# LukasHaas/PIGEON

Hardware: AMD Instinct MI355X
Metric: images/sec end-to-end (ViT+head+refine), 4x336x336 (higher is better)
Workload: dtype f16

## Files before the change

### include/pigeon_hip.h

```cpp
#ifndef PIGEON_HIP_H
#define PIGEON_HIP_H

#include <stddef.h>
#include <stdint.h>

#ifdef __cplusplus
extern "C" {
#endif

#define PG_OK            0
#define PG_EINVAL       -1
#define PG_ENOMEM       -2
#define PG_EHIP         -3
#define PG_ESTATE       -4

#define PG_DTYPE_F32     0
#define PG_DTYPE_BF16    1
#define PG_DTYPE_F16     2
#define PG_DTYPE_F64     3

#define PG_ABI_VERSION   7

const char* pg_last_error(void);
int pg_abi_version(void);
// ... 82 lines not shown
int pg_refine_forward(const pg_bank* bank, const float* q, int B, int P, const double* init_llh,
                      const int64_t* cand, const float* cand_prob, int k, int topk,
                      float temperature, double max_refine_km, float* scratch,
                      float* out_llh, int64_t* out_cell, int32_t* out_choice, void* stream);

int pg_refine_forward_ex(const pg_bank* bank, const float* q, int B, int P, const double* init_llh,
                         const int64_t* cand, const float* cand_prob, int k, int topk, int n_eval,
                         float temperature, double max_refine_km, float* scratch12,
                         float* out_llh, int64_t* out_cell, int32_t* out_choice, int32_t* out_refined, void* stream);

int pg_refine_certainty(const pg_bank* bank, const float* q, int B, int P, const int64_t* cand, const float* cand_prob, int k,
                        int topk, int n_eval, const float* scratch12, const float* W, int C, const float* beta,
                        const float* wstats, float temperature, const int32_t* refined, const int32_t* choice,
                        float* tol, int32_t* code, void* stream);

int pg_requeue_append(const float* head_tol, const float* refine_tol, const int32_t* refine_code, int B, float thr, int force_all,
                      int64_t dst_base, int64_t flushed, int64_t cap, int64_t* counters, int64_t* slot_dst, int32_t* row_slot,
                      uint8_t* certain, int32_t* cause, void* stream);
int pg_rows_to_slots(const void* src, int64_t row_bytes, const int32_t* row_slot, int B, void* dst, void* stream);
int pg_requeue_take(const int64_t* slot_dst, int64_t cap, int64_t head, int n_valid, int n_pad, int64_t* dst_out, void* stream);
int pg_scatter_rows(const void* src, int64_t row_bytes, const int64_t* dst_row, int n, void* dst, int64_t dst_rows,
                    int64_t remap_wb, int64_t remap_b, int64_t remap_off, void* stream);
int pg_head_wstats(const float* W, int C, const float* beta, float* out2, void* stream);

int pg_embedding_debias(float* emb, int64_t n, int dim, const float* bias, void* stream);

typedef struct pg_prep pg_prep;
int pg_prep_create(pg_prep** out, int device, int in_h, int in_w);
int pg_prep_destroy(pg_prep* h);
int pg_prep_geometry(const pg_prep* h, int32_t* out6);
int pg_prep_workspace_bytes(const pg_prep* h, int n_images, size_t* bytes);
int pg_prep_forward(pg_prep* h, const void* images_u8, int n_images, void* out, int out_dtype, void* workspace,
                    size_t workspace_bytes, void* stream);

#define PG_PREP_ITEM_BYTES 80
#define PG_PREP_RAGGED_MAX_IMAGES 65535
typedef struct pg_prep_item {
    uint64_t src_off;
    int32_t in_h, in_w;
    int32_t new_h, new_w, top, left;
    int32_t ksize_h, ksize_v;
    int32_t row0, nrows;
    int32_t tmp_row;
    uint32_t bounds_h_off, kk_h_off, bounds_v_off, kk_v_off;
    int32_t reserved[3];
} pg_prep_item;
// ... 65 lines not shown
```

### pigeon_amd/_lib.py

```python
from __future__ import annotations

import ctypes as C
import os

_HERE = os.path.dirname(os.path.abspath(__file__))
LIB_PATH = os.environ.get("PIGEON_HIP_LIB") or os.path.join(_HERE, "libpigeon_hip.so")

PG_DTYPE_F32, PG_DTYPE_BF16, PG_DTYPE_F16, PG_DTYPE_F64 = 0, 1, 2, 3
EPI_QKV, EPI_GELU, EPI_RESID, EPI_PATCH, EPI_F32, EPI_RESID_STAT, EPI_QKV_LN, EPI_GELU_LN, EPI_GELU_X3 = 0, 1, 2, 3, 4, 5, 6, 7, 8
PROF_CLASSES = ["gemm_qkv", "gemm_out", "gemm_fc1", "gemm_fc2", "gemm_patch", "attention", "layernorm",
                "im2col", "token_mean"]


class PigeonHipError(RuntimeError):
    pass


class VitCfg(C.Structure):
    _fields_ = [("layers", C.c_int32), ("image_size", C.c_int32), ("patch", C.c_int32), ("hidden", C.c_int32),
                ("heads", C.c_int32), ("mlp", C.c_int32), ("ln_eps", C.c_float), ("max_chunk", C.c_int32),
                ("mma_dtype", C.c_int32), ("precise", C.c_int32)]


class Bank(C.Structure):
    _fields_ = [("proto_emb", C.c_void_p), ("cell_off", C.c_void_p), ("proto_lnglat", C.c_void_p),
                ("proto_count", C.c_void_p), ("member_off", C.c_void_p), ("member_idx", C.c_void_p),
                ("train_emb", C.c_void_p), ("train_lnglat", C.c_void_p),
                ("num_cells", C.c_int64), ("num_protos", C.c_int64), ("num_train", C.c_int64)]


class PrepItem(C.Structure):
    _fields_ = [("src_off", C.c_uint64), ("in_h", C.c_int32), ("in_w", C.c_int32), ("new_h", C.c_int32), ("new_w", C.c_int32),
                ("top", C.c_int32), ("left", C.c_int32), ("ksize_h", C.c_int32), ("ksize_v", C.c_int32), ("row0", C.c_int32),
                ("nrows", C.c_int32), ("tmp_row", C.c_int32), ("bounds_h_off", C.c_uint32), ("kk_h_off", C.c_uint32),
                ("bounds_v_off", C.c_uint32), ("kk_v_off", C.c_uint32), ("reserved", C.c_int32 * 3)]


PREP_ITEM_BYTES = 80
assert C.sizeof(PrepItem) == PREP_ITEM_BYTES


_P, _I, _I64, _F, _D, _SZ = C.c_void_p, C.c_int, C.c_int64, C.c_float, C.c_double, C.c_size_t
SIGNATURES = {
    "pg_last_error": (C.c_char_p, []),
    "pg_abi_version": (_I, []),
    "pg_device_count": (_I, []),
    "pg_vit_create": (_I, [C.POINTER(_P), _I, C.POINTER(VitCfg)]),
    "pg_vit_load_weight": (_I, [_P, C.c_char_p, _P, _I, C.POINTER(_I64), _I]),
    "pg_vit_finalize": (_I, [_P]),
    "pg_vit_workspace_bytes": (_I, [_P, _I, C.POINTER(_SZ)]),
    "pg_vit_forward": (_I, [_P, _P, _I, _I, _P, _P, _SZ, _P]),
    "pg_vit_forward_hidden": (_I, [_P, _P, _I, _I, _P, _P, _P, _SZ, _P]),
    "pg_vit_precise_workspace_bytes": (_I, [_P, _I, C.POINTER(_SZ)]),
    "pg_vit_forward_precise": (_I, [_P, _P, _I, _I, _P, _P, _P, _SZ, _P]),
    "pg_vit_graph": (_I, [_P, _I, C.POINTER(_I64), C.POINTER(_I64)]),
    "pg_vit_destroy": (_I, [_P]),
    "pg_vit_mma_dtype": (_I, [_P]),
    "pg_fingerprint": (_I, [_P, _SZ, C.c_uint64, C.POINTER(C.c_uint64), _P]),
    "pg_vit_fingerprint": (_I, [_P, C.POINTER(C.c_uint64)]),
    "pg_vit_profile_enable": (_I, [_P, _I]),
    "pg_vit_profile_read": (_I, [_P, C.POINTER(_I64), C.POINTER(_D)]),
    "pg_vit_profile_reset": (_I, [_P]),
# ... 25 lines not shown
    "pg_prep_ragged_create": (_I, [C.POINTER(_P), _I]),
    "pg_prep_ragged_destroy": (_I, [_P]),
    "pg_prep_ragged_forward": (_I, [_P, _P, _SZ, C.POINTER(PrepItem), _I, _P, _I, _P, _SZ, _P]),
    "pg_proto_build": (_I, [_P, _I, _I64, _P, _P, _I64, _P, _P]),
    "pg_haversine_matrix": (_I, [_P, _I, _P, _I, _I, _P, _P]),
    "pg_haversine_pairs": (_I, [_P, _P, _I, _I64, _P, _P]),
    "pg_smooth_labels": (_I, [_P, _I, _I, _D, _P, _P]),
    "pg_haversine_blocks": (_I, [_P, _P, _P, _I, _D, _P, _P]),
    "pg_optics_graph": (_I, [_P, _P, _P, _I, _I, _P, _P, _P, _P, _P]),
    "pg_optics_plan": (_I, [_I64, _I, C.POINTER(C.c_int32)]),
    "pg_tune_optics_lds_points": (_I, [_I]),
    "pg_head_forward": (_I, [_P, _I, _I, _P, _P, _P, _I, _I, _P, _P, _P, _P, _P, _P]),
    "pg_head_margin": (_I, [_P, _I, _I, _P, _I, _P, _P, _P, _P, _P]),
    "pg_head_certainty": (_I, [_P, _I, _I, _P, _I, _P, _P, _I, _P, _P, _P, _P, _P, _P, _P]),
    "pg_aux_heads_forward": (_I, [_P, _I, _I, _P, _P, _I, _I, _I, _P, _P, _P, _P, _P, _P, _P]),
    "pg_refine_forward": (_I, [C.POINTER(Bank), _P, _I, _I, _P, _P, _P, _I, _I, _F, _D, _P, _P, _P, _P, _P]),
    "pg_refine_forward_ex": (_I, [C.POINTER(Bank), _P, _I, _I, _P, _P, _P, _I, _I, _I, _F, _D, _P, _P, _P, _P, _P, _P]),
    "pg_refine_certainty": (_I, [C.POINTER(Bank), _P, _I, _I, _P, _P, _I, _I, _I, _P, _P, _I, _P, _P, _F, _P, _P, _P, _P, _P]),
    "pg_requeue_append": (_I, [_P, _P, _P, _I, _F, _I, _I64, _I64, _I64, _P, _P, _P, _P, _P, _P]),
    "pg_rows_to_slots": (_I, [_P, _I64, _P, _I, _P, _P]),
    "pg_requeue_take": (_I, [_P, _I64, _I64, _I, _I, _P, _P]),
    "pg_scatter_rows": (_I, [_P, _I64, _P, _I, _P, _I64, _I64, _I64, _I64, _P]),
    "pg_head_wstats": (_I, [_P, _I, _P, _P, _P]),
    "pg_embedding_debias": (_I, [_P, _I64, _I, _P, _P]),
    "pg_op_gemm16": (_I, [_I, _P, _I64, _P, _P, _P, _I64, _I, _I, _I, _I, _F, _I, _P, _I, _P]),
    "pg_op_gemm16_ld": (_I, [_I, _P, _I64, _P, _I64, _P, _P, _I64, _I, _I, _I, _I, _F, _I, _P, _I, _P]),
    "pg_op_rowstat_cast": (_I, [_P, _P, _I, _P, _I64, _F, _P]),
    "pg_op_gemm16_resid_stat": (_I, [_I, _P, _I64, _P, _I64, _P, _P, _I64, _P, _I64, _P, _I, _I, _I, _I, _P]),
    "pg_op_rowstat_finalize": (_I, [_P, _I, _P, _I64, _F, _P]),
    "pg_op_gemm16_ln": (_I, [_I, _P, _I64, _P, _I64, _P, _P, _P, _P, _I64, _I, _I, _I, _I, _F, _I, _I, _P]),
    "pg_op_layernorm": (_I, [_P, _P, _P, _P, _I, _I64, _F, _P]),
    "pg_op_attention": (_I, [_I, _P, _P, _I, _P]),
    "pg_op_im2col": (_I, [_P, _I, _P, _I, _I, _P]),
    "pg_op_token_mean": (_I, [_P, _P, _I, _P]),
    "pg_op_cast_f32": (_I, [_P, _P, _I, _I64, _P]),
    "pg_op_gemm16_parts": (_I, [_I, _P, _I64, _P, _I64, _P, _P, _I, _I, _I, _I, _P]),
    "pg_op_x3_split": (_I, [_P, _P, _I64, _I, _I, _P]),
    "pg_op_x3_layernorm": (_I, [_P, _P, _P, _P, _I64, _F, _P]),
    "pg_op_attention_f32": (_I, [_P, _P, _I, _P]),
    "pg_op_attention_x3": (_I, [_P, _P, _I, _P]),
    "pg_op_x3_im2col": (_I, [_P, _I, _P, _I, _P]),
    "pg_op_sum_parts": (_I, [_P, _I, _I64, _P, _I64, _I, _P]),
    "pg_op_preln": (_I, [_P, _P, _P, _P, _P, _I64, _F, _P, _I, _P, _P]),
    "pg_vit_precise_plan": (_I, [_I, C.POINTER(C.c_int32)]),
}

# ... 35 lines not shown
```

### pigeon_amd/csrc/head.hip

```cpp
#include "common.h"
#include "pigeon_internal.h"
#include "certainty_common.h"
#include <cfloat>

#define HT 64
#define HK 32

__global__ __launch_bounds__(256) void head_logits_kernel(const float* __restrict__ emb, int B, int P,
                                                          const float* __restrict__ W, const float* __restrict__ bias,
                                                          int C, float* __restrict__ logits) {
    __shared__ float As[HK][HT + 1];
    __shared__ float Ws[HK][HT + 1];
    const int tid = threadIdx.x;
    const int c0 = blockIdx.x * HT, b0 = blockIdx.y * HT;
    const int tx = tid & 15, ty = tid >> 4;
    float acc[4][4];
#pragma unroll
    for (int i = 0; i < 4; ++i)
#pragma unroll
        for (int j = 0; j < 4; ++j) acc[i][j] = 0.f;
    const float invP = 1.0f / (float)P;
    for (int k0 = 0; k0 < VIT_HIDDEN; k0 += HK) {
#pragma unroll
        for (int i = 0; i < 8; ++i) {
            const int idx = tid + i * 256;
            const int r = idx >> 5, k = idx & 31;
            float a = 0.f;
            if (b0 + r < B) {
                const float* e = emb + ((int64_t)(b0 + r) * P) * VIT_HIDDEN + k0 + k;
                for (int p = 0; p < P; ++p) a += e[(int64_t)p * VIT_HIDDEN];
                a *= invP;
            }
            As[k][r] = a;
            Ws[k][r] = (c0 + r < C) ? W[(int64_t)(c0 + r) * VIT_HIDDEN + k0 + k] : 0.f;
        }
        __syncthreads();
#pragma unroll
        for (int k = 0; k < HK; ++k) {
            float a[4], w[4];
#pragma unroll
            for (int i = 0; i < 4; ++i) a[i] = As[k][ty * 4 + i];
#pragma unroll
            for (int j = 0; j < 4; ++j) w[j] = Ws[k][tx * 4 + j];
#pragma unroll
            for (int i = 0; i < 4; ++i)
#pragma unroll
                for (int j = 0; j < 4; ++j) acc[i][j] = fmaf(a[i], w[j], acc[i][j]);
        }
        __syncthreads();
    }
#pragma unroll
    for (int i = 0; i < 4; ++i) {
        const int b = b0 + ty * 4 + i;
        if (b >= B) continue;
#pragma unroll
        for (int j = 0; j < 4; ++j) {
            const int c = c0 + tx * 4 + j;
            if (c < C) logits[(int64_t)b * C + c] = acc[i][j] + bias[c];
        }
    }
}

struct ValIdx { float v; int i; };
__device__ __forceinline__ ValIdx block_argbest(ValIdx x, ValIdx* red ) {
#pragma unroll
    for (int o = 32; o >= 1; o >>= 1) {
        const float ov = __shfl_xor(x.v, o, 64);
        const int oi = __shfl_xor(x.i, o, 64);
        if (better(ov, oi, x.v, x.i)) { x.v = ov; x.i = oi; }
    }
    const int wave = threadIdx.x >> 6;
    __syncthreads();
    if ((threadIdx.x & 63) == 0) red[wave] = x;
    __syncthreads();
    ValIdx r = red[0];
#pragma unroll
    for (int w = 1; w < 4; ++w) if (better(red[w].v, red[w].i, r.v, r.i)) r = red[w];
    return r;
}

template <bool GLOBAL>
// ... 35 lines not shown
            topk_val[(int64_t)b * k + r] = best.v;
            topk_idx[(int64_t)b * k + r] = best.i;
            if (r == 0) {
                argmax_out[b] = best.i;
                pred_llh[2 * b] = centroids[2 * (int64_t)best.i];
                pred_llh[2 * b + 1] = centroids[2 * (int64_t)best.i + 1];
            }
            probs[best.i] = -2.f;
        }
        if (GLOBAL) __threadfence_block();
        __syncthreads();
    }
}

extern "C" int pg_head_forward(const float* emb, int B, int P, const float* W, const float* bias,
                               const double* centroids, int C, int k, float* logits, float* topk_val,
                               int64_t* topk_idx, int64_t* argmax, double* pred_llh, void* stream) {
    hipStream_t s = (hipStream_t)stream;
    if (B < 0) { pg_set_error("head: B = %d", B); return PG_EINVAL; }
    if (B == 0) return PG_OK;
    if (!emb || !W || !bias || !centroids || !logits || !topk_val || !topk_idx || !argmax || !pred_llh) {
        pg_set_error("head: null pointer argument"); return PG_EINVAL;
    }
    if (P < 1 || C < 1 || k < 1 || k > C) { pg_set_error("head: bad P=%d C=%d k=%d", P, C, k); return PG_EINVAL; }
    const size_t lds = (size_t)C * sizeof(float);
    const bool big = lds > 150 * 1024;
    dim3 g1((C + HT - 1) / HT, (B + HT - 1) / HT);
    hipLaunchKernelGGL(head_logits_kernel, g1, dim3(256), 0, s, emb, B, P, W, bias, C, logits);
    int rc = pg_check_launch("head_logits");
    if (rc) return rc;
    if (big) {
        float* scratch = nullptr;
        PG_HIP(hipMallocAsync((void**)&scratch, (size_t)B * C * sizeof(float), s));
        hipLaunchKernelGGL(head_row_kernel<true>, dim3(B), dim3(256), 0, s, logits, C, k, centroids, topk_val, topk_idx, argmax, pred_llh, scratch);
        rc = pg_check_launch("head_row (large C)");
        (void)hipFreeAsync(scratch, s);
        return rc;
    }
    static size_t attr_lds = 0;
    if (lds > attr_lds) {
        PG_HIP(hipFuncSetAttribute((const void*)head_row_kernel<false>, hipFuncAttributeMaxDynamicSharedMemorySize, (int)lds));
        attr_lds = lds;
    }
    hipLaunchKernelGGL(head_row_kernel<false>, dim3(B), dim3(256), lds, s, logits, C, k, centroids, topk_val, topk_idx, argmax, pred_llh,
                       (float*)nullptr);
    return pg_check_launch("head_row");
}

__global__ __launch_bounds__(256) void head_margin_kernel(const float* __restrict__ logits, int C, const float* __restrict__ emb, int P,
                                                          const float* __restrict__ W, float* __restrict__ margin,
                                                          float* __restrict__ sens, int64_t* __restrict__ top2) {
// ... 56 lines not shown
```

### pigeon_amd/csrc/requeue.hip

```cpp
#include "common.h"
#include "pigeon_internal.h"

namespace {

__global__ void __launch_bounds__(256)
requeue_append_kernel(const float* __restrict__ head_tol, const float* __restrict__ refine_tol, const int32_t* __restrict__ refine_code,
                      int B, float thr, int force_all, int64_t dst_base, int64_t flushed, int64_t cap,
                      int64_t* __restrict__ counters, int64_t* __restrict__ slot_dst, int32_t* __restrict__ row_slot,
                      uint8_t* __restrict__ certain, int32_t* __restrict__ cause) {
    __shared__ int wave_cnt[4];
    __shared__ int64_t s_app, s_drop;
    const int tid = threadIdx.x, lane = tid & 63, wv = tid >> 6;
    if (tid == 0) { s_app = counters ? counters[0] : 0; s_drop = counters ? counters[1] : 0; }
    __syncthreads();
    for (int base = 0; base < B; base += 256) {
        const int r = base + tid;
        bool flag = false;
        int why = 0;
        if (r < B) {
            const bool h_unc = force_all || !(head_tol[r] > thr);
            const bool r_unc = refine_tol ? !(refine_tol[r] > thr) : false;
            flag = h_unc || r_unc;
            why = h_unc ? 1 : (r_unc ? (refine_code ? refine_code[r] : 2) : 0);
            if (r_unc && !h_unc && why == 0) why = 2;
// ... 74 lines not shown
head_wstats_kernel(const float* __restrict__ W, int C, const float* __restrict__ beta, unsigned int* __restrict__ out) {
    const int lane = threadIdx.x & 63;
    const int c = blockIdx.x * 4 + (threadIdx.x >> 6);
    if (c >= C) return;
    const float* row = W + (int64_t)c * 1024;
    float n2 = 0.f, wb = 0.f;
#pragma unroll
    for (int i = 0; i < 4; ++i) {
        const f32x4 v = *(const f32x4*)(row + i * 256 + lane * 4);
        n2 = fmaf(v[0], v[0], fmaf(v[1], v[1], fmaf(v[2], v[2], fmaf(v[3], v[3], n2))));
        if (beta) {
            const f32x4 b = *(const f32x4*)(beta + i * 256 + lane * 4);
            wb = fmaf(v[0], b[0], fmaf(v[1], b[1], fmaf(v[2], b[2], fmaf(v[3], b[3], wb))));
        }
    }
    n2 = wave_sum(n2);
    wb = wave_sum(wb);
    if (lane == 0) {
        atomicMax(out + 0, __float_as_uint(sqrtf(n2)));
        atomicMax(out + 1, __float_as_uint(fabsf(wb)));
    }
}

int vec_bytes(const void* a, const void* b, int64_t row_bytes) {
    const uintptr_t al = (uintptr_t)a | (uintptr_t)b | (uintptr_t)row_bytes;
    return (al & 15) == 0 ? 16 : (al & 7) == 0 ? 8 : (al & 3) == 0 ? 4 : 1;
}
dim3 row_grid(int64_t row_bytes, int vb, int rows) {
    int64_t chunks = (row_bytes / vb + 256 * 8 - 1) / (256 * 8);
    if (chunks < 1) chunks = 1;
    if (chunks > 256) chunks = 256;
    return dim3((unsigned)chunks, (unsigned)rows, 1);
}

}

extern "C" int pg_requeue_append(const float* head_tol, const float* refine_tol, const int32_t* refine_code, int B, float thr,
                                 int force_all, int64_t dst_base, int64_t flushed, int64_t cap, int64_t* counters, int64_t* slot_dst,
                                 int32_t* row_slot, uint8_t* certain, int32_t* cause, void* stream) {
    if (B < 0 || cap < 0) { pg_set_error("requeue_append: B = %d, cap = %lld", B, (long long)cap); return PG_EINVAL; }
    if (B == 0) return PG_OK;
    if (!head_tol) { pg_set_error("requeue_append: null head_tol"); return PG_EINVAL; }
    if (cap > 0 && (!counters || !slot_dst || !row_slot)) { pg_set_error("requeue_append: a queue needs counters, slot_dst and row_slot"); return PG_EINVAL; }
    hipLaunchKernelGGL(requeue_append_kernel, dim3(1), dim3(256), 0, (hipStream_t)stream, head_tol, refine_tol, refine_code, B, thr,
                       force_all, dst_base, flushed, cap, counters, slot_dst, row_slot, certain, cause);
    return pg_check_launch("requeue_append_kernel");
// ... 18 lines not shown
                               int64_t remap_wb, int64_t remap_b, int64_t remap_off, void* stream) {
    if (n < 0 || row_bytes < 0 || dst_rows < 0) { pg_set_error("scatter_rows: bad size"); return PG_EINVAL; }
    if (n == 0 || row_bytes == 0) return PG_OK;
    if (!src || !dst_row || !dst) { pg_set_error("scatter_rows: null argument"); return PG_EINVAL; }
    if (n > 65535) { pg_set_error("scatter_rows: n = %d rows exceed the launch grid (65535)", n); return PG_EINVAL; }
    const int vb = vec_bytes(src, dst, row_bytes);
    const dim3 g = row_grid(row_bytes, vb, n);
    hipStream_t s = (hipStream_t)stream;
#define PG_SCATTER(V) hipLaunchKernelGGL(scatter_rows_kernel<V>, g, dim3(256), 0, s, (const char*)src, row_bytes, dst_row, (char*)dst, \
                                         dst_rows, remap_wb, remap_b, remap_off)
    if (vb == 16) PG_SCATTER(uint4); else if (vb == 8) PG_SCATTER(uint2); else if (vb == 4) PG_SCATTER(uint32_t); else PG_SCATTER(uint8_t);
#undef PG_SCATTER
    return pg_check_launch("scatter_rows_kernel");
}

extern "C" int pg_requeue_take(const int64_t* slot_dst, int64_t cap, int64_t head, int n_valid, int n_pad, int64_t* dst_out, void* stream) {
    if (n_pad < 0 || n_valid < 0 || n_valid > n_pad || cap <= 0 || head < 0) { pg_set_error("requeue_take: bad argument"); return PG_EINVAL; }
    if (n_pad == 0) return PG_OK;
    if (!slot_dst || !dst_out) { pg_set_error("requeue_take: null argument"); return PG_EINVAL; }
    hipLaunchKernelGGL(requeue_take_kernel, dim3((n_pad + 255) / 256), dim3(256), 0, (hipStream_t)stream, slot_dst, cap, head, n_valid, n_pad, dst_out);
    return pg_check_launch("requeue_take_kernel");
}

extern "C" int pg_head_wstats(const float* W, int C, const float* beta, float* out2, void* stream) {
    if (C < 0) { pg_set_error("head_wstats: C = %d", C); return PG_EINVAL; }
    if (!out2 || (C > 0 && !W)) { pg_set_error("head_wstats: null argument"); return PG_EINVAL; }
    hipStream_t s = (hipStream_t)stream;
    PG_HIP(hipMemsetAsync(out2, 0, 2 * sizeof(float), s));
    if (C == 0) return PG_OK;
    hipLaunchKernelGGL(head_wstats_kernel, dim3((C + 3) / 4), dim3(256), 0, s, W, C, beta, (unsigned int*)out2);
    return pg_check_launch("head_wstats_kernel");
}
```

### pigeon_amd/deferred.py

```python
from __future__ import annotations

from collections import deque
from typing import Dict, List, Optional

import torch

from .utils import TopK


AUX_KEYS = ('aux_preds', 'aux_cls', 'aux_tol', 'aux_code')


class LocalComm:
    rank, world_size = 0, 1

    def gather_many(self, tensors, out=None):
        if out is None:
            return list(tensors)
        for t, o in zip(tensors, out):
            o.copy_(t)
        return list(out)


class DeferredExact:
# ... 50 lines not shown
        self.cap = 0
        self.q_pixels = self.slot_dst = None
        self.counters = torch.zeros((2,), dtype=torch.int64, device=dev)
        self.counts_all = torch.zeros((R, W), dtype=torch.int64, device=dev)
        self.host_counts = torch.zeros((R, W), dtype=torch.int64)
        if dev.type == 'cuda':
            self.host_counts = self.host_counts.pin_memory()
            self.events = [torch.cuda.Event() for _ in range(R)]
        else:
            self.events = [None] * R
        self.flushed = [0] * W
        self.px_shape = None

    def _alloc_queue(self, px_rows: torch.Tensor):
        if self.pass_quantum is None:
            self.pass_quantum = round_quantum(px_rows)
            if self._min_flush_arg is None:
                self.min_flush = self.pass_quantum or 10
        self.cap = (self.B if self.immediate else self.min_flush + (self.pass_quantum or 0) + 2 * self.B)
        self.q_pixels = torch.zeros((self.cap,) + tuple(px_rows.shape[1:]), dtype=px_rows.dtype, device=px_rows.device)
        self.slot_dst = torch.zeros((self.cap,), dtype=torch.int64, device=px_rows.device)
        self._true_cap = torch.ones((self.cap,), dtype=torch.bool, device=px_rows.device)
        self.px_shape = (tuple(px_rows.shape[1:]), px_rows.dtype)

    def _mark(self, m):
        if m is None:
            return
        if self.dev.type == 'cuda':
            ev = torch.cuda.Event(enable_timing=True)
            ev.record()
            m.append(ev)
        else:
            import time
            m.append(time.perf_counter())

    @torch.no_grad()
    def submit(self, pixel_values=None, embedding=None, index=None, meta=None) -> List[dict]:
        model, comm, ops = self.model, self.comm, self.ops
        marks = [] if self.marks is not None else None
        settled = []
        if self.dev is None:
            self.dev = model.cell_layer.weight.device
        self._mark(marks)
        st = model.encode_head(pixel_values, embedding)
        b = int(st['tol'].shape[0])
        px = st.get('pixel_values')
# ... 5 lines not shown
            self.pending.append(dict(step=self.n_submitted, slot=-1, b=0, meta=meta, appended=None, can_fix=False, ready=empty))
            self.n_submitted += 1
            return self._advance(final=False)
        can_fix = bool(getattr(model, 'exact_top1', False)) and px is not None and not st.get('exact_tier', False)
        if self.ring is not None and (b > self.B or (comm.world_size > 1 and b != self.B)):
            out = self.flush()
            self.ring = None
            st['pixel_values'] = None
            return out + self.submit(pixel_values, embedding, index, meta)
        if self.ring is None:
            self._alloc(st, b)
        rank, B, WB = comm.rank, self.B, self.WB
        step = self.n_submitted
        slot = step % self.R
        if any(r['slot'] == slot for r in self.pending):
            raise RuntimeError('DeferredExact: result ring overrun (max_lag too large for the ring)')
        gbase, lbase = slot * WB, slot * B
        dev = self.dev
        if index is None:
            index = self._arange[:b] if rank == 0 else self._arange[:b] + rank * b
        index = index.to(dev)
        exact_tier = bool(st.get('exact_tier', False))
        thr = st['thr']
        for k, buf in self.local.items():
            if k in st:
                buf[lbase:lbase + b].copy_(st[k])
        ring = self.ring
        slab = lambda k: ring[k][gbase:gbase + comm.world_size * b]
        own = slice(gbase + rank * b, gbase + (rank + 1) * b)
        self._mark(marks)
        comm.gather_many([st['embedding'], st['topk_indices'], st['topk_values'], st['preds_LLH'], st['preds_geocell'], index],
                         out=[slab('embedding'), slab('topk_indices'), slab('topk_values'), slab('preds_LLH'), slab('preds_geocell'),
                              slab('index')])
        self._mark(marks)
        rtol = rcode = None
        W_head = model.cell_layer.weight.data
        if self.refiner is not None:
            llh_r, cell_r, rtol, rcode, self.boundary_checked = self.refiner.forward_certain(
                ring['embedding'][own], ring['preds_LLH'][own], ring['topk_indices'][own], ring['topk_values'][own], W_head,
                st['wstats'], st.get('drift'))
            self.local['refine_tol'][lbase:lbase + b].copy_(rtol)
            self.local['refine_code'][lbase:lbase + b].copy_(rcode)
        wants_queue = bool(getattr(model, 'exact_top1', False)) and px is not None
        if wants_queue:
            px_rows = px.reshape((b, -1)).contiguous()
            if self.q_pixels is None or self.px_shape != (tuple(px_rows.shape[1:]), px_rows.dtype):
                if self.q_pixels is not None:
                    settled = self.flush()
                    self.counters.zero_()
                    self.flushed = [0] * comm.world_size
                    self._prev_appended = [0] * comm.world_size
                self._alloc_queue(px_rows)
        if can_fix:
            certain, cause, row_slot = ops.requeue_append(st['tol'], rtol, rcode, thr, False, dst_base=gbase + rank * b,
                                                          flushed=self.flushed[rank], cap=self.cap, counters=self.counters,
                                                          slot_dst=self.slot_dst)
            ops.rows_to_slots(px_rows, row_slot, self.q_pixels)
        else:
            certain, cause, _ = ops.requeue_append(st['tol'], rtol, rcode, thr, False)
        small = [certain.view(torch.bool), cause, (self._true if exact_tier else self._false)[:b], self.counters[:1]]
        outs = [slab('certain'), slab('cause'), slab('exact'), self.counts_all[slot]]
        if self.refiner is not None:
            small += [llh_r, cell_r]
            outs += [slab('refined_LLH'), slab('refined_geocell')]
        self._mark(marks)
        comm.gather_many(small, out=outs)
        self.host_counts[slot].copy_(self.counts_all[slot], non_blocking=True)
        if self.events[slot] is not None:
            self.events[slot].record()
        self._mark(marks)
        if marks is not None:
            self.marks.append(marks)
        self.pending.append(dict(step=step, slot=slot, b=b, meta=meta, appended=None, can_fix=can_fix))
        self.n_submitted += 1
        st['pixel_values'] = None
        return settled + self._advance(final=False)

    def flush(self) -> List[dict]:
        return self._advance(final=True)

    def _empty_result(self, st: dict, index, meta) -> dict:
        dev = st['tol'].device
        k = int(getattr(self.model, 'num_candidates', st['topk_indices'].shape[1]))
        z = lambda dt, *shape: torch.zeros((0,) + shape, dtype=dt, device=dev)
        state = {kk: st[kk] for kk in ('embedding', 'topk_values', 'topk_indices', 'preds_LLH', 'preds_geocell', 'tol', 'margin', 'sens',
                                       'logits') + AUX_KEYS if kk in st}
        state.update(certain=z(torch.bool), exact=z(torch.bool), cause=z(torch.int32), pixel_values=None)
        res = dict(embedding=st['embedding'], topk_indices=st['topk_indices'][:, :k], topk_values=st['topk_values'][:, :k],
                   preds_LLH=st['preds_LLH'], preds_geocell=st['preds_geocell'], index=z(torch.int64), certain=z(torch.bool),
# ... 97 lines not shown
            if k in sx:
                ops.scatter_rows(sx[k], dst, buf, remap=(self.WB, self.B, rank * self.B))
        for r in range(W):
            self.flushed[r] += lens[r]
        self._mark(span)
        self.flush_log.append(dict(at_step=at_step, queued=list(lens), slots_run=n_pad, span=span))

    def exact_pass_ms(self, entries=None) -> List[float]:
        out = []
        for f in (self.flush_log if entries is None else entries):
            sp = f.get('span')
            if sp:
                out.append((sp[1] - sp[0]) * 1e3 if isinstance(sp[0], float) else sp[0].elapsed_time(sp[1]))
        return out

    def _emit(self, rec: dict) -> dict:
        if 'ready' in rec:
            return rec['ready']
        comm = self.comm
        rank, b = comm.rank, rec['b']
        gbase, lbase = rec['slot'] * self.WB, rec['slot'] * self.B
        n = comm.world_size * b
        ring = self.ring
        res = {k: ring[k][gbase:gbase + n].clone() for k in ring}
        k = int(getattr(self.model, 'num_candidates', res['topk_indices'].shape[1]))
        own = slice(rank * b, (rank + 1) * b)
        state = {'embedding': res['embedding'][own], 'topk_values': res['topk_values'][own], 'topk_indices': res['topk_indices'][own],
                 'preds_LLH': res['preds_LLH'][own], 'preds_geocell': res['preds_geocell'][own],
                 'certain': res['certain'][own], 'exact': res['exact'][own], 'cause': res['cause'][own], 'pixel_values': None}
        if self.refiner is not None:
            state['refined_LLH'], state['refined_geocell'] = res['refined_LLH'][own], res['refined_geocell'][own]
        for kk, buf in self.local.items():
            state[kk] = buf[lbase:lbase + b].clone()
        res['topk_indices'] = res['topk_indices'][:, :k]
        res['topk_values'] = res['topk_values'][:, :k]
        prev = self._prev_appended
        res['queued'] = [a - p for a, p in zip(rec['appended'], prev)]
        self._prev_appended = rec['appended']
        res['step'], res['meta'], res['state'] = rec['step'], rec['meta'], state
        return res

    def check_nothing_dropped(self) -> int:
        return int(self.counters[1].item()) if self.ring is not None else 0


def round_quantum(px_rows: torch.Tensor, tokens: int = 577, panel_rows: int = 256, n_tiles: int = 4) -> int:
    if px_rows.device.type != 'cuda':
        return 0
    cus = torch.cuda.get_device_properties(px_rows.device).multi_processor_count
    images = (cus // n_tiles) * panel_rows // tokens
    views = max(1, int(px_rows.shape[1]) // (3 * 336 * 336))
    return max(1, images // views)


def as_model_output(model, res: dict, labels=None, labels_clf=None, labels_multi_task=None, labels_climate=None, labels_month=None):
    if labels_multi_task is None and labels_climate is None and labels_month is None:
# ... 6 lines not shown
```

### pigeon_amd/hip_ops.py

```python
from __future__ import annotations

import ctypes as C
from typing import Dict, Optional

import torch

from . import _lib
from ._lib import Bank, VitCfg, check, load

TOKENS, HIDDEN, MLP, PATCHES, KPAD = 577, 1024, 4096, 576, 640


def _p(t: Optional[torch.Tensor]):
    return C.c_void_p(0) if t is None else C.c_void_p(t.data_ptr())


def _stream():
    return C.c_void_p(torch.cuda.current_stream().cuda_stream)


_T16 = {torch.float16: _lib.PG_DTYPE_F16, torch.bfloat16: _lib.PG_DTYPE_BF16}
_PIXDT = {torch.float32: _lib.PG_DTYPE_F32, torch.float16: _lib.PG_DTYPE_F16, torch.bfloat16: _lib.PG_DTYPE_BF16}
_PG2T = {_lib.PG_DTYPE_F16: torch.float16, _lib.PG_DTYPE_BF16: torch.bfloat16, _lib.PG_DTYPE_F32: torch.float32}

# ... 645 lines not shown


def requeue_take(slot_dst: torch.Tensor, head: int, n_valid: int, n_pad: int) -> torch.Tensor:
    _dev(slot_dst, torch.int64)
    out = torch.empty((n_pad,), dtype=torch.int64, device=slot_dst.device)
    check(load().pg_requeue_take(_p(slot_dst), slot_dst.numel(), int(head), int(n_valid), int(n_pad), _p(out), _stream()), "pg_requeue_take")
    return out


def scatter_rows(src: torch.Tensor, dst_row: torch.Tensor, dst: torch.Tensor, remap=None) -> None:
    _dev(src); _dev(dst); _dev(dst_row, torch.int64)
    n = src.shape[0]
    _shape(dst_row, "dst_row", n)
    if src.dtype != dst.dtype or tuple(src.shape[1:]) != tuple(dst.shape[1:]):
        raise _lib.PigeonHipError(f"scatter_rows: rows of {src.dtype} {tuple(src.shape[1:])} into {dst.dtype} {tuple(dst.shape[1:])}")
    rb = 1
    for d in src.shape[1:]:
        rb *= int(d)
    rb *= src.element_size()
    wb, b, off = remap if remap is not None else (0, 0, 0)
    check(load().pg_scatter_rows(_p(src), rb, _p(dst_row), n, _p(dst), dst.shape[0], int(wb), int(b), int(off), _stream()), "pg_scatter_rows")


def x3_split(x: torch.Tensor, gelu: bool = False) -> torch.Tensor:
    _dev(x, torch.float32)
    rows, cols = x.shape
    y = torch.empty((rows, 3 * cols), dtype=torch.float16, device=x.device)
    check(load().pg_op_x3_split(_p(x), _p(y), rows, cols, 1 if gelu else 0, _stream()), "pg_op_x3_split")
    return y


def gemm16_parts(A: torch.Tensor, W: torch.Tensor, bias: Optional[torch.Tensor], S: int) -> torch.Tensor:
    _dev(A); _dev(W)
    if W.dtype != A.dtype or A.shape[1] != W.shape[1] or A.shape[1] % S:
        raise _lib.PigeonHipError("gemm16_parts: A and W must share dtype and a K' divisible by S")
    M, Kt = A.shape
    N = W.shape[0]
    out = torch.empty((S, M, N), dtype=torch.float32, device=A.device)
    check(load().pg_op_gemm16_parts(_dt16(A), _p(A), A.stride(0), _p(W), W.stride(0), _p(bias), _p(out), M, N, Kt // S, S, _stream()),
          "pg_op_gemm16_parts")
    return out


def x3_layernorm(x: torch.Tensor, gamma: torch.Tensor, beta: torch.Tensor, eps: float = 1e-5) -> torch.Tensor:
    _dev(x, torch.float32)
    rows = x.numel() // HIDDEN
# ... 202 lines not shown
```

Before: 2529.

## Batch ring copies into one kernel and rewrite head logits as wave-dot kernel

Adds a descriptor-table copy kernel, exposed as ring_store and ring_release, that replaces many small per-tensor copy_/clone/gather launches in the deferred ring with a single launch per batch of up to 32 blocks. For single-process communicators the gathers are skipped and folded into that batched copy, with release outputs packed into one allocation. Separately, the head logits kernel is rewritten so each wave keeps four class weight rows in registers, token-means the embeddings into LDS, and reduces dot products with cross-lane shuffles instead of the old shared-memory tiled GEMM. The goal is lower launch and host overhead on the small-batch path, at the cost of more complex code, and the new head kernel loops over every batch row inside each block.

```diff
diff --git a/include/pigeon_hip.h b/include/pigeon_hip.h
--- a/include/pigeon_hip.h
+++ b/include/pigeon_hip.h
@@ -128,6 +128,18 @@
 int pg_scatter_rows(const void* src, int64_t row_bytes, const int64_t* dst_row, int n, void* dst, int64_t dst_rows,
                     int64_t remap_wb, int64_t remap_b, int64_t remap_off, void* stream);
 int pg_head_wstats(const float* W, int C, const float* beta, float* out2, void* stream);
+
+#define PG_RING_MAX_DESC 32
+typedef struct pg_ring_desc {
+    const void* src;
+    void*       dst;
+    int64_t     row_bytes;
+    int64_t     src_row;
+    int64_t     dst_row;
+    int64_t     rows;
+} pg_ring_desc;
+int pg_ring_store(const pg_ring_desc* desc, int n, void* stream);
+int pg_ring_release(const pg_ring_desc* desc, int n, void* stream);
 
 int pg_embedding_debias(float* emb, int64_t n, int dim, const float* bias, void* stream);
 
diff --git a/pigeon_amd/_lib.py b/pigeon_amd/_lib.py
--- a/pigeon_amd/_lib.py
+++ b/pigeon_amd/_lib.py
@@ -38,6 +38,11 @@
 
 PREP_ITEM_BYTES = 80
 assert C.sizeof(PrepItem) == PREP_ITEM_BYTES
+
+
+class RingDesc(C.Structure):
+    _fields_ = [("src", C.c_void_p), ("dst", C.c_void_p), ("row_bytes", C.c_int64), ("src_row", C.c_int64), ("dst_row", C.c_int64),
+                ("rows", C.c_int64)]
 
 
 _P, _I, _I64, _F, _D, _SZ = C.c_void_p, C.c_int, C.c_int64, C.c_float, C.c_double, C.c_size_t
@@ -109,6 +114,8 @@
     "pg_requeue_take": (_I, [_P, _I64, _I64, _I, _I, _P, _P]),
     "pg_scatter_rows": (_I, [_P, _I64, _P, _I, _P, _I64, _I64, _I64, _I64, _P]),
     "pg_head_wstats": (_I, [_P, _I, _P, _P, _P]),
+    "pg_ring_store": (_I, [C.POINTER(RingDesc), _I, _P]),
+    "pg_ring_release": (_I, [C.POINTER(RingDesc), _I, _P]),
     "pg_embedding_debias": (_I, [_P, _I64, _I, _P, _P]),
     "pg_op_gemm16": (_I, [_I, _P, _I64, _P, _P, _P, _I64, _I, _I, _I, _I, _F, _I, _P, _I, _P]),
     "pg_op_gemm16_ld": (_I, [_I, _P, _I64, _P, _I64, _P, _P, _I64, _I, _I, _I, _I, _F, _I, _P, _I, _P]),
diff --git a/pigeon_amd/csrc/head.hip b/pigeon_amd/csrc/head.hip
--- a/pigeon_amd/csrc/head.hip
+++ b/pigeon_amd/csrc/head.hip
@@ -3,60 +3,74 @@
 #include "certainty_common.h"
 #include <cfloat>
 
-#define HT 64
-#define HK 32
-
-__global__ __launch_bounds__(256) void head_logits_kernel(const float* __restrict__ emb, int B, int P,
-                                                          const float* __restrict__ W, const float* __restrict__ bias,
-                                                          int C, float* __restrict__ logits) {
-    __shared__ float As[HK][HT + 1];
-    __shared__ float Ws[HK][HT + 1];
-    const int tid = threadIdx.x;
-    const int c0 = blockIdx.x * HT, b0 = blockIdx.y * HT;
-    const int tx = tid & 15, ty = tid >> 4;
-    float acc[4][4];
-#pragma unroll
-    for (int i = 0; i < 4; ++i)
-#pragma unroll
-        for (int j = 0; j < 4; ++j) acc[i][j] = 0.f;
+#define HL_WAVES 8
+#define HL_WR 4
+#define HL_ROWS 16
+
+__global__ __launch_bounds__(HL_WAVES * 64, 4) void head_logits_kernel(const float* __restrict__ emb, int B, int P,
+                                                                    const float* __restrict__ W, const float* __restrict__ bias,
+                                                                    int C, float* __restrict__ logits) {
+    __shared__ __attribute__((aligned(16))) float am[HL_ROWS][VIT_HIDDEN];
+    const int tid = threadIdx.x, lane = tid & 63, wave = tid >> 6;
+    const int c0 = (blockIdx.x * HL_WAVES + wave) * HL_WR;
+    f32x4 w[HL_WR][4];
+#pragma unroll
+    for (int j = 0; j < HL_WR; ++j) {
+        const int c = c0 + j < C ? c0 + j : C - 1;
+        ld16(W + (int64_t)c * VIT_HIDDEN, lane, w[j]);
+    }
     const float invP = 1.0f / (float)P;
-    for (int k0 = 0; k0 < VIT_HIDDEN; k0 += HK) {
-#pragma unroll
-        for (int i = 0; i < 8; ++i) {
-            const int idx = tid + i * 256;
-            const int r = idx >> 5, k = idx & 31;
-            float a = 0.f;
-            if (b0 + r < B) {
-                const float* e = emb + ((int64_t)(b0 + r) * P) * VIT_HIDDEN + k0 + k;
-                for (int p = 0; p < P; ++p) a += e[(int64_t)p * VIT_HIDDEN];
-                a *= invP;
-            }
-            As[k][r] = a;
-            Ws[k][r] = (c0 + r < C) ? W[(int64_t)(c0 + r) * VIT_HIDDEN + k0 + k] : 0.f;
+    const int col = (tid & 255) * 4, rhalf = tid >> 8;
+    const bool b3 = (lane & 8) != 0, b4 = (lane & 16) != 0, b5 = (lane & 32) != 0;
+    for (int b0 = 0; b0 < B; b0 += HL_ROWS) {
+        const int nb = B - b0 < HL_ROWS ? B - b0 : HL_ROWS;
+        if (b0) __syncthreads();
+#pragma unroll 1
+        for (int h = 0; h < HL_ROWS; h += HL_ROWS / 2) {
+            f32x4 acc[HL_ROWS / 4];
+            const float* src = emb + (int64_t)b0 * P * VIT_HIDDEN + col;
+            int off[HL_ROWS / 4];
+#pragma unroll
+            for (int i = 0; i < HL_ROWS / 4; ++i) {
+                const int r = h + rhalf + 2 * i;
+                acc[i] = (f32x4){0.f, 0.f, 0.f, 0.f};
+                off[i] = (r < nb ? r : nb - 1) * P * VIT_HIDDEN;
+            }
+            for (int p = 0; p < P; ++p, src += VIT_HIDDEN) {
+#pragma unroll
+                for (int i = 0; i < HL_ROWS / 4; ++i) acc[i] += *(const f32x4*)(src + off[i]);
+            }
+#pragma unroll
+            for (int i = 0; i < HL_ROWS / 4; ++i) *(f32x4*)&am[h + rhalf + 2 * i][col] = acc[i] * invP;
         }
         __syncthreads();
-#pragma unroll
-        for (int k = 0; k < HK; ++k) {
-            float a[4], w[4];
-#pragma unroll
-            for (int i = 0; i < 4; ++i) a[i] = As[k][ty * 4 + i];
-#pragma unroll
-            for (int j = 0; j < 4; ++j) w[j] = Ws[k][tx * 4 + j];
-#pragma unroll
-            for (int i = 0; i < 4; ++i)
-#pragma unroll
-                for (int j = 0; j < 4; ++j) acc[i][j] = fmaf(a[i], w[j], acc[i][j]);
-        }
-        __syncthreads();
-    }
-#pragma unroll
-    for (int i = 0; i < 4; ++i) {
-        const int b = b0 + ty * 4 + i;
-        if (b >= B) continue;
-#pragma unroll
-        for (int j = 0; j < 4; ++j) {
-            const int c = c0 + tx * 4 + j;
-            if (c < C) logits[(int64_t)b * C + c] = acc[i][j] + bias[c];
+        for (int r = 0; r < nb; r += 2) {
+            const int r1 = r + 1 < nb ? r + 1 : r;
+            f32x4 a0[4], a1[4];
+            ld16(am[r], lane, a0);
+            ld16(am[r1], lane, a1);
+            float v[2 * HL_WR];
+#pragma unroll
+            for (int j = 0; j < HL_WR; ++j) {
+                float s0 = 0.f, s1 = 0.f;
+#pragma unroll
+                for (int i = 0; i < 4; ++i)
+#pragma unroll
+                    for (int e = 0; e < 4; ++e) { s0 = fmaf(a0[i][e], w[j][i][e], s0); s1 = fmaf(a1[i][e], w[j][i][e], s1); }
+                v[j] = s0; v[HL_WR + j] = s1;
+            }
+            float t[4], u[2];
+#pragma unroll
+            for (int i = 0; i < 4; ++i) t[i] = (b5 ? v[2 * i + 1] : v[2 * i]) + __shfl_xor(b5 ? v[2 * i] : v[2 * i + 1], 32, 64);
+#pragma unroll
+            for (int i = 0; i < 2; ++i) u[i] = (b4 ? t[2 * i + 1] : t[2 * i]) + __shfl_xor(b4 ? t[2 * i] : t[2 * i + 1], 16, 64);
+            float x = (b3 ? u[1] : u[0]) + __shfl_xor(b3 ? u[0] : u[1], 8, 64);
+            x += __shfl_xor(x, 4, 64);
+            x += __shfl_xor(x, 2, 64);
+            x += __shfl_xor(x, 1, 64);
+            const int q = (b3 ? 4 : 0) + (b4 ? 2 : 0) + (b5 ? 1 : 0);
+            const int rr = q / HL_WR, c = c0 + q % HL_WR;
+            if ((lane & 7) == 0 && r + rr < nb && c < C) logits[(int64_t)(b0 + r + rr) * C + c] = x + bias[c];
         }
     }
 }
@@ -138,11 +152,11 @@
     if (!emb || !W || !bias || !centroids || !logits || !topk_val || !topk_idx || !argmax || !pred_llh) {
         pg_set_error("head: null pointer argument"); return PG_EINVAL;
     }
-    if (P < 1 || C < 1 || k < 1 || k > C) { pg_set_error("head: bad P=%d C=%d k=%d", P, C, k); return PG_EINVAL; }
+    if (P < 1 || P > 65535 || C < 1 || k < 1 || k > C) { pg_set_error("head: bad P=%d C=%d k=%d", P, C, k); return PG_EINVAL; }
     const size_t lds = (size_t)C * sizeof(float);
     const bool big = lds > 150 * 1024;
-    dim3 g1((C + HT - 1) / HT, (B + HT - 1) / HT);
-    hipLaunchKernelGGL(head_logits_kernel, g1, dim3(256), 0, s, emb, B, P, W, bias, C, logits);
+    const int cells = HL_WAVES * HL_WR;
+    hipLaunchKernelGGL(head_logits_kernel, dim3((C + cells - 1) / cells), dim3(HL_WAVES * 64), 0, s, emb, B, P, W, bias, C, logits);
     int rc = pg_check_launch("head_logits");
     if (rc) return rc;
     if (big) {
diff --git a/pigeon_amd/csrc/requeue.hip b/pigeon_amd/csrc/requeue.hip
--- a/pigeon_amd/csrc/requeue.hip
+++ b/pigeon_amd/csrc/requeue.hip
@@ -1,5 +1,7 @@
 #include "common.h"
 #include "pigeon_internal.h"
+#include <cstdint>
+#include <cstdio>
 
 namespace {
 
@@ -120,6 +122,55 @@
     }
 }
 
+struct RingTable { pg_ring_desc d[PG_RING_MAX_DESC]; };
+
+template <typename V>
+__device__ __forceinline__ void copy_bytes(const char* __restrict__ src, char* __restrict__ dst, int64_t bytes) {
+    const int64_t n = bytes / (int64_t)sizeof(V);
+    const V* s = (const V*)src;
+    V* d = (V*)dst;
+    for (int64_t i = (int64_t)blockIdx.x * blockDim.x + threadIdx.x; i < n; i += (int64_t)gridDim.x * blockDim.x) d[i] = s[i];
+}
+
+__global__ void __launch_bounds__(256) ring_copy_kernel(const RingTable t) {
+    const pg_ring_desc d = t.d[blockIdx.y];
+    const int64_t bytes = d.rows * d.row_bytes;
+    const char* src = (const char*)d.src + d.src_row * d.row_bytes;
+    char* dst = (char*)d.dst + d.dst_row * d.row_bytes;
+    const uintptr_t al = (uintptr_t)src | (uintptr_t)dst | (uintptr_t)bytes;
+    if ((al & 15) == 0) copy_bytes<uint4>(src, dst, bytes);
+    else if ((al & 7) == 0) copy_bytes<uint2>(src, dst, bytes);
+    else if ((al & 3) == 0) copy_bytes<uint32_t>(src, dst, bytes);
+    else copy_bytes<uint8_t>(src, dst, bytes);
+}
+
+int ring_copy(const char* what, const pg_ring_desc* desc, int n, hipStream_t s) {
+    if (n < 0) { pg_set_error("%s: n = %d", what, n); return PG_EINVAL; }
+    if (n > 0 && !desc) { pg_set_error("%s: null table", what); return PG_EINVAL; }
+    for (int i0 = 0; i0 < n; i0 += PG_RING_MAX_DESC) {
+        RingTable t;
+        int m = 0;
+        int64_t most = 0;
+        for (int i = i0; i < n && i < i0 + PG_RING_MAX_DESC; ++i) {
+            const pg_ring_desc& d = desc[i];
+            if (d.row_bytes < 0 || d.rows < 0 || d.src_row < 0 || d.dst_row < 0) { pg_set_error("%s: entry %d has a negative size or row", what, i); return PG_EINVAL; }
+            if (d.rows == 0 || d.row_bytes == 0) continue;
+            if (!d.src || !d.dst) { pg_set_error("%s: entry %d has a null pointer", what, i); return PG_EINVAL; }
+            if (d.rows > INT64_MAX / d.row_bytes) { pg_set_error("%s: entry %d overflows", what, i); return PG_EINVAL; }
+            t.d[m++] = d;
+            if (d.rows * d.row_bytes > most) most = d.rows * d.row_bytes;
+        }
+        if (m == 0) continue;
+        for (int i = m; i < PG_RING_MAX_DESC; ++i) t.d[i] = pg_ring_desc{nullptr, nullptr, 0, 0, 0, 0};
+        int64_t chunks = (most + 256 * 16 - 1) / (256 * 16);
+        if (chunks > 64) chunks = 64;
+        hipLaunchKernelGGL(ring_copy_kernel, dim3((unsigned)chunks, (unsigned)m), dim3(256), 0, s, t);
+        const int rc = pg_check_launch("ring_copy_kernel");
+        if (rc) return rc;
+    }
+    return PG_OK;
+}
+
 int vec_bytes(const void* a, const void* b, int64_t row_bytes) {
     const uintptr_t al = (uintptr_t)a | (uintptr_t)b | (uintptr_t)row_bytes;
     return (al & 15) == 0 ? 16 : (al & 7) == 0 ? 8 : (al & 3) == 0 ? 4 : 1;
@@ -184,6 +235,14 @@
     return pg_check_launch("requeue_take_kernel");
 }
 
+extern "C" int pg_ring_store(const pg_ring_desc* desc, int n, void* stream) {
+    return ring_copy("ring_store", desc, n, (hipStream_t)stream);
+}
+
+extern "C" int pg_ring_release(const pg_ring_desc* desc, int n, void* stream) {
+    return ring_copy("ring_release", desc, n, (hipStream_t)stream);
+}
+
 extern "C" int pg_head_wstats(const float* W, int C, const float* beta, float* out2, void* stream) {
     if (C < 0) { pg_set_error("head_wstats: C = %d", C); return PG_EINVAL; }
     if (!out2 || (C > 0 && !W)) { pg_set_error("head_wstats: null argument"); return PG_EINVAL; }
diff --git a/pigeon_amd/deferred.py b/pigeon_amd/deferred.py
--- a/pigeon_amd/deferred.py
+++ b/pigeon_amd/deferred.py
@@ -96,6 +96,15 @@
         self.slot_dst = torch.zeros((self.cap,), dtype=torch.int64, device=px_rows.device)
         self._true_cap = torch.ones((self.cap,), dtype=torch.bool, device=px_rows.device)
         self.px_shape = (tuple(px_rows.shape[1:]), px_rows.dtype)
+
+    @staticmethod
+    def _put(store, src: torch.Tensor, dst: torch.Tensor, row: int):
+        if store is None:
+            dst[row:row + src.shape[0]].copy_(src)
+            return
+        if src.dtype != dst.dtype:
+            src = src.to(dst.dtype)
+        store.append((src.contiguous(), dst, row))
 
     def _mark(self, m):
         if m is None:
@@ -147,25 +156,33 @@
         index = index.to(dev)
         exact_tier = bool(st.get('exact_tier', False))
         thr = st['thr']
+        store = [] if hasattr(ops, 'ring_store') else None
+        fused = store is not None and type(comm) is LocalComm
         for k, buf in self.local.items():
             if k in st:
-                buf[lbase:lbase + b].copy_(st[k])
+                self._put(store, st[k], buf, lbase)
         ring = self.ring
         slab = lambda k: ring[k][gbase:gbase + comm.world_size * b]
         own = slice(gbase + rank * b, gbase + (rank + 1) * b)
+        first = ('embedding', 'topk_indices', 'topk_values', 'preds_LLH', 'preds_geocell')
         self._mark(marks)
-        comm.gather_many([st['embedding'], st['topk_indices'], st['topk_values'], st['preds_LLH'], st['preds_geocell'], index],
-                         out=[slab('embedding'), slab('topk_indices'), slab('topk_values'), slab('preds_LLH'), slab('preds_geocell'),
-                              slab('index')])
+        if fused:
+            for k in first:
+                self._put(store, st[k], ring[k], gbase)
+            self._put(store, index, ring['index'], gbase)
+            mine = {k: st[k] for k in first}
+        else:
+            comm.gather_many([st[k] for k in first] + [index], out=[slab(k) for k in first] + [slab('index')])
+            mine = {k: ring[k][own] for k in first}
         self._mark(marks)
         rtol = rcode = None
         W_head = model.cell_layer.weight.data
         if self.refiner is not None:
             llh_r, cell_r, rtol, rcode, self.boundary_checked = self.refiner.forward_certain(
-                ring['embedding'][own], ring['preds_LLH'][own], ring['topk_indices'][own], ring['topk_values'][own], W_head,
+                mine['embedding'], mine['preds_LLH'], mine['topk_indices'], mine['topk_values'], W_head,
                 st['wstats'], st.get('drift'))
-            self.local['refine_tol'][lbase:lbase + b].copy_(rtol)
-            self.local['refine_code'][lbase:lbase + b].copy_(rcode)
+            self._put(store, rtol, self.local['refine_tol'], lbase)
+            self._put(store, rcode, self.local['refine_code'], lbase)
         wants_queue = bool(getattr(model, 'exact_top1', False)) and px is not None
         if wants_queue:
             px_rows = px.reshape((b, -1)).contiguous()
@@ -184,12 +201,19 @@
         else:
             certain, cause, _ = ops.requeue_append(st['tol'], rtol, rcode, thr, False)
         small = [certain.view(torch.bool), cause, (self._true if exact_tier else self._false)[:b], self.counters[:1]]
-        outs = [slab('certain'), slab('cause'), slab('exact'), self.counts_all[slot]]
+        keys = ['certain', 'cause', 'exact']
         if self.refiner is not None:
             small += [llh_r, cell_r]
-            outs += [slab('refined_LLH'), slab('refined_geocell')]
+            keys += ['refined_LLH', 'refined_geocell']
         self._mark(marks)
-        comm.gather_many(small, out=outs)
+        if fused:
+            for k, t in zip(keys, small[:3] + small[4:]):
+                self._put(store, t, ring[k], gbase)
+            self._put(store, small[3].view(1, 1), self.counts_all, slot)
+        else:
+            comm.gather_many(small, out=[slab(k) for k in keys[:3]] + [self.counts_all[slot]] + [slab(k) for k in keys[3:]])
+        if store:
+            ops.ring_store(store)
         self.host_counts[slot].copy_(self.counts_all[slot], non_blocking=True)
         if self.events[slot] is not None:
             self.events[slot].record()
@@ -333,7 +357,13 @@
         gbase, lbase = rec['slot'] * self.WB, rec['slot'] * self.B
         n = comm.world_size * b
         ring = self.ring
-        res = {k: ring[k][gbase:gbase + n].clone() for k in ring}
+        if hasattr(self.ops, 'ring_release'):
+            out = self.ops.ring_release([(ring[k], gbase, n) for k in ring] + [(buf, lbase, b) for buf in self.local.values()])
+            res = dict(zip(ring, out))
+            mine = dict(zip(self.local, out[len(ring):]))
+        else:
+            res = {k: ring[k][gbase:gbase + n].clone() for k in ring}
+            mine = {kk: buf[lbase:lbase + b].clone() for kk, buf in self.local.items()}
         k = int(getattr(self.model, 'num_candidates', res['topk_indices'].shape[1]))
         own = slice(rank * b, (rank + 1) * b)
         state = {'embedding': res['embedding'][own], 'topk_values': res['topk_values'][own], 'topk_indices': res['topk_indices'][own],
@@ -341,8 +371,7 @@
                  'certain': res['certain'][own], 'exact': res['exact'][own], 'cause': res['cause'][own], 'pixel_values': None}
         if self.refiner is not None:
             state['refined_LLH'], state['refined_geocell'] = res['refined_LLH'][own], res['refined_geocell'][own]
-        for kk, buf in self.local.items():
-            state[kk] = buf[lbase:lbase + b].clone()
+        state.update(mine)
         res['topk_indices'] = res['topk_indices'][:, :k]
         res['topk_values'] = res['topk_values'][:, :k]
         prev = self._prev_appended
diff --git a/pigeon_amd/hip_ops.py b/pigeon_amd/hip_ops.py
--- a/pigeon_amd/hip_ops.py
+++ b/pigeon_amd/hip_ops.py
@@ -691,6 +691,50 @@
     check(load().pg_scatter_rows(_p(src), rb, _p(dst_row), n, _p(dst), dst.shape[0], int(wb), int(b), int(off), _stream()), "pg_scatter_rows")
 
 
+def _ring_table(what: str, blocks):
+    tab = (_lib.RingDesc * max(len(blocks), 1))()
+    for i, (src, src_row, dst, dst_row, rows) in enumerate(blocks):
+        _dev(src); _dev(dst)
+        if src.dtype != dst.dtype or tuple(src.shape[1:]) != tuple(dst.shape[1:]) or src.dim() < 1:
+            raise _lib.PigeonHipError(f"{what}: rows of {src.dtype} {tuple(src.shape[1:])} into {dst.dtype} {tuple(dst.shape[1:])}")
+        if rows < 0 or src_row < 0 or dst_row < 0 or src_row + rows > src.shape[0] or dst_row + rows > dst.shape[0]:
+            raise _lib.PigeonHipError(f"{what}: rows [{src_row}, {src_row + rows}) of {src.shape[0]} into [{dst_row}, {dst_row + rows}) "
+                                      f"of {dst.shape[0]}")
+        rb = src.element_size()
+        for d in src.shape[1:]:
+            rb *= int(d)
+        tab[i] = _lib.RingDesc(src.data_ptr(), dst.data_ptr(), rb, int(src_row), int(dst_row), int(rows))
+    return tab
+
+
+def ring_store(blocks) -> None:
+    blocks = [(s, 0, d, r, int(s.shape[0])) for s, d, r in blocks]
+    check(load().pg_ring_store(_ring_table("ring_store", blocks), len(blocks), _stream()), "pg_ring_store")
+
+
+_RELEASE_ALIGN = 16
+
+
+def ring_release(blocks) -> list:
+    if not blocks:
+        return []
+    sizes = []
+    for s, _, rows in blocks:
+        nb = int(rows) * s.element_size()
+        for d in s.shape[1:]:
+            nb *= int(d)
+        sizes.append(nb)
+    offs, total = [], 0
+    for nb in sizes:
+        offs.append(total)
+        total += (nb + _RELEASE_ALIGN - 1) // _RELEASE_ALIGN * _RELEASE_ALIGN
+    packed = torch.empty((max(total, _RELEASE_ALIGN),), dtype=torch.uint8, device=blocks[0][0].device)
+    outs = [packed[o:o + nb].view(s.dtype).view((int(rows),) + tuple(s.shape[1:])) for (s, _, rows), o, nb in zip(blocks, offs, sizes)]
+    table = [(s, r0, o, 0, int(rows)) for (s, r0, rows), o in zip(blocks, outs)]
+    check(load().pg_ring_release(_ring_table("ring_release", table), len(table), _stream()), "pg_ring_release")
+    return outs
+
+
 def x3_split(x: torch.Tensor, gelu: bool = False) -> torch.Tensor:
     _dev(x, torch.float32)
     rows, cols = x.shape
```

Measured after the change: 2537, median of 6. Within noise of the previous version (+0.3%).
